# team-charls/charls

Measured on AMD Instinct MI355X. Metric: MPixels/s encode+decode, 4096x4096 8-bit gray, bit-exact vs CharLS, higher is better.
Workload: dtype u8

## Files before the change

charls_amd/batch.py:

```python
from __future__ import annotations

import ctypes as C
from dataclasses import dataclass

import numpy as np

from . import capi


class CodecParams(C.Structure):
    _fields_ = [("frame_info", capi.FrameInfo), ("near_lossless", C.c_int32), ("interleave_mode", C.c_int32),
                ("color_transformation", C.c_int32), ("preset_coding_parameters", capi.PcParameters),
                ("encoding_options", C.c_uint32), ("restart_interval", C.c_uint32)]


class DeviceShard(C.Structure):
    _fields_ = [("device", C.c_int32), ("frame_count", C.c_uint32), ("d_frames", C.c_void_p), ("d_streams", C.c_void_p),
                ("hip_stream", C.c_void_p)]


class Gather(C.Structure):
    _fields_ = [("root_shard", C.c_uint32), ("d_gathered", C.c_void_p), ("capacity_bytes", C.c_size_t),
                ("offsets", C.POINTER(C.c_uint64)), ("total_bytes", C.POINTER(C.c_uint64)), ("transport", C.c_int32)]


TRANSPORT_AUTO, TRANSPORT_RCCL, TRANSPORT_PEER_COPIES = 0, 1, 2


def _bind(lib):
    l = lib.lib
    if getattr(l, "_batch_bound", False):
        return l
    l.charls_amd_encode_batch_device.argtypes = [C.POINTER(CodecParams), C.c_uint32, C.c_void_p, C.c_size_t, C.c_uint32,
                                                 C.c_void_p, C.c_size_t, C.POINTER(C.c_uint64), C.POINTER(C.c_int32),
                                                 C.c_void_p]
    l.charls_amd_encode_batch_device.restype = C.c_int32
    l.charls_amd_decode_batch_device.argtypes = [C.c_uint32, C.c_void_p, C.c_size_t, C.POINTER(C.c_uint64), C.c_void_p,
                                                 C.c_size_t, C.c_uint32, C.POINTER(CodecParams), C.POINTER(C.c_int32),
                                                 C.c_void_p]
    l.charls_amd_decode_batch_device.restype = C.c_int32
    l.charls_amd_last_timings.argtypes = [C.POINTER(C.c_double), C.c_int32]
    l.charls_amd_last_timings.restype = C.c_int32
    l.charls_amd_set_encode_engine.argtypes = [C.c_int32]
    l.charls_amd_set_encode_engine.restype = C.c_int32
    l.charls_amd_set_workspace_limit.argtypes = [C.c_uint64]
    l.charls_amd_set_workspace_limit.restype = C.c_int32
    l.charls_amd_release_work_areas.argtypes = []
    l.charls_amd_release_work_areas.restype = C.c_int32
    l.charls_amd_work_area_bytes.argtypes = []
    l.charls_amd_work_area_bytes.restype = C.c_uint64
    l.charls_amd_encode_batch_devices.argtypes = [C.POINTER(CodecParams), C.c_uint32, C.POINTER(DeviceShard), C.c_size_t,
                                                  C.c_uint32, C.c_size_t, C.POINTER(C.c_uint64), C.POINTER(C.c_int32),
                                                  C.POINTER(Gather)]
    l.charls_amd_encode_batch_devices.restype = C.c_int32
    l.charls_amd_decode_batch_devices.argtypes = [C.c_uint32, C.POINTER(DeviceShard), C.c_size_t, C.POINTER(C.c_uint64),
                                                  C.c_size_t, C.c_uint32, C.POINTER(CodecParams), C.POINTER(C.c_int32)]
    l.charls_amd_decode_batch_devices.restype = C.c_int32
    u64p, i32p, u32p = C.POINTER(C.c_uint64), C.POINTER(C.c_int32), C.POINTER(C.c_uint32)
    l.charls_amd_index_size_bound.argtypes = [C.POINTER(CodecParams), C.c_uint32, C.POINTER(C.c_size_t)]
    l.charls_amd_index_size_bound.restype = C.c_int32
    l.charls_amd_decode_batch_device_and_index.argtypes = [C.c_uint32, C.c_void_p, C.c_size_t, u64p, C.c_void_p, C.c_size_t, C.c_uint32,
                                                           C.c_uint32, C.c_void_p, C.c_size_t, u64p, C.POINTER(CodecParams), i32p,
                                                           C.c_void_p]
    l.charls_amd_decode_batch_device_and_index.restype = C.c_int32
    l.charls_amd_decode_batch_device_indexed.argtypes = [C.c_uint32, C.c_void_p, C.c_size_t, u64p, C.c_void_p, C.c_size_t, u64p,
                                                         C.c_void_p, C.c_size_t, C.c_uint32, C.POINTER(CodecParams), i32p, C.c_void_p]
    l.charls_amd_decode_batch_device_indexed.restype = C.c_int32
    l.charls_amd_decode_rows_batch_device.argtypes = [C.c_uint32, C.c_void_p, C.c_size_t, u64p, C.c_void_p, C.c_size_t, u64p, u32p, u32p,
                                                      C.c_void_p, C.c_size_t, C.c_uint32, i32p, C.c_void_p]
    l.charls_amd_decode_rows_batch_device.restype = C.c_int32
    l.charls_amd_index_counters.argtypes = [u64p, C.c_int32]
    l.charls_amd_index_counters.restype = C.c_int32
    l._batch_bound = True
    return l


def estimated_destination_size(width, height, bits, components) -> int:
    raw = width * height * components * ((bits + 7) // 8)
    return raw + raw // 16 + 1024 + 34


@dataclass
class EncodedBatch:
    streams: "torch.Tensor"
    sizes: np.ndarray
    errcs: np.ndarray
    gpu_ms: tuple


def last_timings(lib=None):
    l = _bind(lib or capi.load_product())
    buf = (C.c_double * 8)()
    n = l.charls_amd_last_timings(buf, 8)
    return tuple(buf[i] for i in range(n))


def encode_batch(frames, *, bits_per_sample=8, component_count=1, interleave_mode=0, near_lossless=0,
                 color_transformation=0, preset=(0, 0, 0, 0, 0), encoding_options=0, restart_interval=0, streams=None,
                 lib=None) -> EncodedBatch:
    import torch
    lib = lib or capi.load_product()
    l = _bind(lib)
    assert frames.is_cuda and frames.is_contiguous()
    count = frames.shape[0]
    if component_count == 1 or interleave_mode == 0:
        height, width = frames.shape[-2], frames.shape[-1]
    else:
        height, width = frames.shape[1], frames.shape[2]
    frame_pitch = frames[0].numel() * frames.element_size()
    if streams is None:
        pitch = (estimated_destination_size(width, height, bits_per_sample, component_count) + 255) & ~255
        streams = torch.empty((count, pitch), dtype=torch.uint8, device=frames.device)
    assert streams.is_contiguous() and streams.shape[0] == count
    p = CodecParams(capi.FrameInfo(width, height, bits_per_sample, component_count), near_lossless, interleave_mode,
                    color_transformation, capi.PcParameters(*preset), encoding_options, restart_interval)
    sizes = np.zeros(count, dtype=np.uint64)
    errcs = np.zeros(count, dtype=np.int32)
    stream = torch.cuda.current_stream(frames.device).cuda_stream
    rc = l.charls_amd_encode_batch_device(C.byref(p), count, frames.data_ptr(), frame_pitch, 0, streams.data_ptr(),
                                          streams.shape[1], sizes.ctypes.data_as(C.POINTER(C.c_uint64)),
                                          errcs.ctypes.data_as(C.POINTER(C.c_int32)), C.c_void_p(stream))
    if rc != 0:
        raise capi.JpegLSError(rc, "charls_amd_encode_batch_device")
    return EncodedBatch(streams, sizes, errcs, last_timings(lib))


def decode_batch(streams, sizes, out, *, lib=None):
    import torch
    lib = lib or capi.load_product()
    l = _bind(lib)
    assert streams.is_cuda and streams.is_contiguous() and out.is_cuda and out.is_contiguous()
    count = streams.shape[0]
    sizes = np.ascontiguousarray(sizes, dtype=np.uint64)
    errcs = np.zeros(count, dtype=np.int32)
    p = CodecParams()
    frame_pitch = out[0].numel() * out.element_size()
    stream = torch.cuda.current_stream(streams.device).cuda_stream
    rc = l.charls_amd_decode_batch_device(count, streams.data_ptr(), streams.shape[1],
                                          sizes.ctypes.data_as(C.POINTER(C.c_uint64)), out.data_ptr(), frame_pitch, 0,
                                          C.byref(p), errcs.ctypes.data_as(C.POINTER(C.c_int32)), C.c_void_p(stream))
    if rc != 0:
        raise capi.JpegLSError(rc, "charls_amd_decode_batch_device")
    return p, errcs, last_timings(lib)



def index_size_bound(width, height, bits_per_sample=8, component_count=1, interleave_mode=0, near_lossless=0,
# ... 237 lines not shown
```

charls_amd/csrc/device/knobs.h:

```cpp
#pragma once
#include <atomic>
#include <climits>
#include <cstdlib>
#include <cstring>
#include <mutex>

namespace jls::knobs {

enum Knob : int
{
    kDecodeGroup = 0,
    kExactDecoder,
    kSequentialIntervals,
    kBlockStuffing,
    kSpecStuffing,
    kJobEvents,
    kWarmEvents,
    kRunJobEvents,
    kRunWarmEvents,
    kRareWarmEvents,
    kTileSamples,
    kPixelMode,
    kSpecChunk,
    kSpecWarm,
    kBatchRounds,
    kCoalesce,
    kCoalesceWaitUs,
    kDecodeWavesPerCu,
    kDecodeWorkgroupWaves,
    kTrace,
    kIdleReleaseMs,
    kNearDecodePixels,
    kCount
};

constexpr long long kUnset = LLONG_MIN;

inline const char* name_of(int k)
{
    static const char* const names[kCount] = {"DECODE_GROUP", "EXACT_DECODER", "SEQUENTIAL_INTERVALS", "BLOCK_STUFFING", "SPEC_STUFFING",
                                              "JOB_EVENTS", "WARM_EVENTS", "RUN_JOB_EVENTS", "RUN_WARM_EVENTS", "RARE_WARM_EVENTS",
                                              "TILE_SAMPLES", "PIXEL_MODE", "SPEC_CHUNK", "SPEC_WARM", "BATCH_ROUNDS", "COALESCE",
                                              "COALESCE_WAIT_US", "DECODE_WAVES_PER_CU", "DECODE_WORKGROUP_WAVES", "TRACE", "IDLE_RELEASE_MS", "NEAR_DECODE_PIXELS"};
    return k >= 0 && k < kCount ? names[k] : nullptr;
}

struct Table
{
    std::atomic<long long> value[kCount];
};

inline long long from_environment(int k)
{
    char name[64] = "CHARLS_AMD_";
    std::strncat(name, name_of(k), sizeof name - std::strlen(name) - 1);
    const char* env = std::getenv(name);
    if (env == nullptr)
        return kUnset;
    return *env == '\0' ? 1 : std::atoll(env);
}

inline Table& table()
{
    static Table* t = [] {
        auto* fresh = new Table;
        for (int k = 0; k < kCount; ++k)
#ifdef JLS_KNOBS_LIVE_ENV
            fresh->value[k].store(kUnset, std::memory_order_relaxed);
#else
            fresh->value[k].store(from_environment(k), std::memory_order_relaxed);
#endif
        return fresh;
    }();
    return *t;
}

inline long long get(Knob k)
{
    const long long v = table().value[k].load(std::memory_order_relaxed);
#ifdef JLS_KNOBS_LIVE_ENV
    if (v == kUnset)
        return from_environment(k);
#endif
    return v;
}

inline bool is_set(Knob k)
{
    return get(k) != kUnset;
}

inline long long get_or(Knob k, long long otherwise)
{
    const long long v = get(k);
    return v == kUnset ? otherwise : v;
}
// ... 18 lines not shown
```

charls_amd/csrc/device/runtime.h:

```cpp
#pragma once
#include <hip/hip_runtime_api.h>

#include <cstddef>
#include <cstdint>

#include "../host/common.h"
#include "scan_types.h"

namespace jls::dev {

charls_jpegls_errc device_status() noexcept;
void require_device();

inline void hip_check(hipError_t e)
{
    if (e != hipSuccess)
        raise(e == hipErrorOutOfMemory ? CHARLS_JPEGLS_ERRC_NOT_ENOUGH_MEMORY : CHARLS_AMD_ERRC_DEVICE_FAILURE);
}

class DeviceBuffer
{
public:
    DeviceBuffer() = default;
    DeviceBuffer(const DeviceBuffer&) = delete;
// ... 85 lines not shown
void launch_find_scan_end(const uint8_t* slots, const MarkerSearch* searches, unsigned long long* found, uint32_t count, hipStream_t stream);
void launch_place_plane_scans(uint8_t* slots, uint64_t slot_pitch, const uint8_t* headers, uint32_t header_size, uint32_t rounds,
                              const uint8_t* private_streams, uint64_t capacity, const ScanResult* results, FrameCursorPod* cursors,
                              uint32_t* redo, uint32_t frames, hipStream_t stream);
void launch_place_epilogue(uint8_t* slots, uint64_t slot_pitch, FrameCursorPod* cursors, bool even_size, uint64_t* sizes,
                           uint32_t* errcs, uint32_t frames, hipStream_t stream);

void set_workspace_limit(uint64_t bytes) noexcept;
uint64_t workspace_limit() noexcept;
void release_shared_work_areas() noexcept;
size_t shared_work_area_bytes() noexcept;
DeviceBuffer& plane_arena();
constexpr int kSeekArenas = 6;
DeviceBuffer& seek_arena(int which);
void* try_ensure(DeviceBuffer& buffer, size_t bytes) noexcept;
void release_work_areas() noexcept;
size_t work_area_bytes() noexcept;
size_t thread_work_area_bytes() noexcept;
void release_thread_work_areas() noexcept;
size_t work_area_budget() noexcept;
uint64_t pipeline_fallback_scans() noexcept;
uint64_t exact_retry_scans() noexcept;

inline size_t with_headroom(size_t bytes) noexcept
{
    size_t v = size_t{64} << 10;
    while (v < bytes)
        v <<= 1;
    return v;
}
size_t shared_areas_keep_bytes() noexcept;

class SharedAreasScope
{
public:
    SharedAreasScope();
    ~SharedAreasScope();
    SharedAreasScope(const SharedAreasScope&) = delete;
    SharedAreasScope& operator=(const SharedAreasScope&) = delete;
    size_t bytes() const noexcept;
    void release() noexcept;

private:
    int device_{0};
};

struct Timings
{
    double values[8];
    int32_t count;
};
Timings& last_timings() noexcept;

constexpr int tile_counter_count = 6;
void speculation_counters(uint64_t out[tile_counter_count]) noexcept;

}
```

charls_amd/csrc/device/runtime.hip:

```cpp
#include <hip/hip_runtime.h>

#include <atomic>
#include <cstdlib>
#include <cstring>
#include <mutex>
#include <vector>

#include "knobs.h"
#include "runtime.h"
#include "scan_serial.hip"
#include "container_kernels.hip"
#include "scan_wave_decode.hip"
#include "pipeline_common.hip"
#include "block_stuffing.hip"
#include "speculative_stuffing.hip"
#include "tile_pipeline.hip"
#include "scan_fast_decode.hip"
#include "scan_group_decode.hip"
#include "group_launch.h"
#include "restart_intervals.hip"
#include "seek_decode.h"

namespace jls::dev {

namespace {
std::once_flag g_once;
charls_jpegls_errc g_status = CHARLS_AMD_ERRC_DEVICE_UNAVAILABLE;
std::atomic<int32_t> g_engine{0};
std::atomic<uint64_t> g_workspace_limit{0};

void probe() noexcept
{
    int count = 0;
    if (hipGetDeviceCount(&count) != hipSuccess || count <= 0)
    {
        (void)hipGetLastError();
        return;
    }
    int device = 0;
    if (hipGetDevice(&device) != hipSuccess)
        return;
    hipDeviceProp_t prop;
    if (hipGetDeviceProperties(&prop, device) != hipSuccess)
        return;
    if (std::strncmp(prop.gcnArchName, "gfx950", 6) != 0 && std::getenv("CHARLS_AMD_ALLOW_ANY_ARCH") == nullptr)
        return;
    g_status = CHARLS_JPEGLS_ERRC_SUCCESS;
}
}

charls_jpegls_errc device_status() noexcept
{
    std::call_once(g_once, probe);
    return g_status;
}

void require_device()
{
    if (device_status() != CHARLS_JPEGLS_ERRC_SUCCESS)
        raise(CHARLS_AMD_ERRC_DEVICE_UNAVAILABLE);
}
// ... 374 lines not shown
        retry_descs[slot] = descs[i];
    }
}

__global__ void scatter_retries(const ScanResult* __restrict__ retry_results, const uint32_t* __restrict__ retry_index,
                                uint32_t retries, ScanResult* __restrict__ results)
{
    const uint32_t s = blockIdx.x * blockDim.x + threadIdx.x;
    if (s < retries)
        results[retry_index[s]] = retry_results[s];
}

template <typename S>
void launch_wave_decode(int nc, const ScanDesc* d_descs, ScanResult* d_results, uint32_t count, size_t lds,
                        hipStream_t stream)
{
    switch (nc)
    {
    case 1:
        hipLaunchKernelGGL((decode_scans_wave<S, 1>), dim3(count), dim3(64), lds, stream, d_descs, d_results);
        break;
    case 2:
        hipLaunchKernelGGL((decode_scans_wave<S, 2>), dim3(count), dim3(64), lds, stream, d_descs, d_results);
        break;
    case 3:
        hipLaunchKernelGGL((decode_scans_wave<S, 3>), dim3(count), dim3(64), lds, stream, d_descs, d_results);
        break;
    default:
        hipLaunchKernelGGL((decode_scans_wave<S, 4>), dim3(count), dim3(64), lds, stream, d_descs, d_results);
        break;
    }
}
}

bool seek_decode_eligible(const ScanDesc& d) noexcept
{
    return d.restart_interval == 0 && wave_decode_eligible(d);
}

uint64_t decode_launch_key(const ScanDesc& d) noexcept
{
    const uint64_t base = (static_cast<uint64_t>(d.width) << 16) | (static_cast<uint64_t>(d.components & 0xFF) << 8) |
                          (static_cast<uint64_t>(d.interleave_mode & 3) << 4) | (d.near_lossless != 0 ? 8u : 0u) |
                          (fast_decode_eligible(d) || pixel_group_lanes(d, 1) != 0 ? 4u : 0u) |
                          (d.bits_per_sample > 8 ? 2u : 0u) | (wave_decode_eligible(d) ? 1u : 0u);
    if (!interval_decode_candidate(d))
        return base;
    return (uint64_t{1} << 63) | (static_cast<uint64_t>(d.restart_interval) << 47) | (static_cast<uint64_t>(d.height) << 31) |
           (static_cast<uint64_t>(d.width & 0xFFFF) << 15) | (static_cast<uint64_t>(d.components & 7) << 12) |
           (static_cast<uint64_t>(d.interleave_mode & 3) << 10) | (base & 15u);
}

namespace {
constexpr int kMaxPipelineLanes = 2;
struct PipelineLanes
{
    hipStream_t streams[kMaxPipelineLanes]{};
    bool created = false;
    int device = -1;
    ~PipelineLanes() { destroy(); }
    void destroy() noexcept
    {
        if (!created)
            return;
        int current = 0;
        const bool switched = hipGetDevice(&current) == hipSuccess && current != device && hipSetDevice(device) == hipSuccess;
        for (hipStream_t s : streams)
            (void)hipStreamDestroy(s);
        if (switched)
            (void)hipSetDevice(current);
        created = false;
    }
    void ensure()
    {
        int current = 0;
        hip_check(hipGetDevice(&current));
        if (created && current == device)
            return;
        destroy();
        for (hipStream_t& s : streams)
            hip_check(hipStreamCreateWithFlags(&s, hipStreamNonBlocking));
        created = true;
        device = current;
    }
};

constexpr int kIntervalArenas = 8;
struct WorkAreas
{
    DeviceBuffer pipeline, plane, interval[kIntervalArenas], seek[kSeekArenas];
    PipelineLanes lanes;
    size_t bytes() const noexcept
    {
        size_t total = pipeline.capacity() + plane.capacity();
        for (const DeviceBuffer& b : interval)
            total += b.capacity();
        for (const DeviceBuffer& b : seek)
            total += b.capacity();
        return total;
    }
    void release() noexcept
    {
        pipeline.release();
        plane.release();
        for (DeviceBuffer& b : interval)
            b.release();
        for (DeviceBuffer& b : seek)
// ... 391 lines not shown
            o = align_up(o + n, 256);
            return at;
        };
        off_keyinv = take(samples * 2);
        off_seg = take(static_cast<size_t>(tiles + 1) * pipe::kChains * 4);
        off_total = take(pipe::kChains * 4);
        off_base = take(pipe::kChains * 4);
        off_jobfirst = take((pipe::kChains + 1) * 4);
        off_planpart = take(static_cast<size_t>(tile::kPlanGroups) * pipe::kChains * 4);
        const uint32_t run_slots = d.bits_per_sample > 8 ? 1u : 2u;
        const size_t slot_bytes = d.bits_per_sample > 8 ? 4 : 2;
        const size_t slots = static_cast<size_t>(tile::slots_capacity(samples, run_slots, lines)) + tile::kSlack;
        off_rec = take(slots * slot_bytes);
        off_code = take(slots * slot_bytes);
        off_jobs = take(max_jobs * sizeof(tile::JobState));
        off_runjobs = take(max_run_jobs * sizeof(tile::RunJob));
        off_bbase = take(static_cast<size_t>(tiles) * 16);
        off_raw = take(raw_bytes);
        off_bits = take(16);
        off_status = take(8);
        off_stuff = take(std::max(block_stuffing_enabled() ? (raw_bytes / pipe::kStuffChunk + 1) * pipe::kStuffWords * 4 : 0,
                                  spec_stuffing_enabled() ? pipe::stuff_spec_table_words(raw_bytes, pipe::stuff_spec_geometry().chunk_bytes) * 4 : 0));
        bytes = o;
    }
};

void ensure_tile_attributes()
{
    static std::mutex guard;
    static uint64_t done[4] = {0, 0, 0, 0};
    int device = 0;
    hip_check(hipGetDevice(&device));
    std::lock_guard<std::mutex> lock(guard);
    if (device >= 0 && device < 256 && (done[device >> 6] >> (device & 63) & 1u) != 0)
        return;
    const int lds = 160 * 1024;
    auto set = [&](const void* kernel) { hip_check(hipFuncSetAttribute(kernel, hipFuncAttributeMaxDynamicSharedMemorySize, lds)); };
    set(reinterpret_cast<const void*>(tile::analyze_tiles<uint8_t, 0>));
    set(reinterpret_cast<const void*>(tile::analyze_tiles<uint16_t, 0>));
    set(reinterpret_cast<const void*>(tile::pack_tiles<uint8_t>));
    set(reinterpret_cast<const void*>(tile::pack_tiles<uint16_t>));
    set(reinterpret_cast<const void*>(tile::sort_tiles<uint8_t, 0>));
    set(reinterpret_cast<const void*>(tile::sort_tiles<uint16_t, 0>));
    set(reinterpret_cast<const void*>(tile::analyze_pixel_tiles<uint8_t>));
    set(reinterpret_cast<const void*>(tile::analyze_pixel_tiles<uint16_t>));
    set(reinterpret_cast<const void*>(tile::sort_pixel_tiles<uint8_t>));
    set(reinterpret_cast<const void*>(tile::sort_pixel_tiles<uint16_t>));
    if (device >= 0 && device < 256)
        done[device >> 6] |= uint64_t{1} << (device & 63);
}

constexpr size_t kCounterBytes = 256;

template <typename S>
void run_tile_pipeline(const ScanDesc& proto, ScanDesc* d_descs, ScanResult* d_results, uint32_t count, hipStream_t stream)
{
    const size_t budget = t_shared_areas != nullptr ? std::min(arena_budget(pipeline_arena().capacity()), shared_areas_keep_bytes())
                                                    : arena_budget(pipeline_arena().capacity());
    TileLayout lay(proto, proto.stream_capacity, count);
    size_t per_scan = lay.bytes + 2 * (sizeof(tile::Work) + sizeof(pipe::Work));
    uint32_t resident = static_cast<uint32_t>(std::max<size_t>(1, std::min<size_t>(count, budget / per_scan)));
    if (resident < count)
    {
        lay = TileLayout(proto, proto.stream_capacity, resident);
        per_scan = lay.bytes + 2 * (sizeof(tile::Work) + sizeof(pipe::Work));
        resident = static_cast<uint32_t>(std::max<size_t>(1, std::min<size_t>(count, budget / per_scan)));
    }
    uint8_t* arena = nullptr;
    const bool over_limit = g_workspace_limit.load() != 0 && budget < per_scan;
    for (; !over_limit;)
    {
        uint32_t room = resident;
        if (t_shared_areas != nullptr)
        {
            room = 1;
            while (room < resident)
                room *= 2;
            room = static_cast<uint32_t>(std::max<size_t>(resident, std::min<size_t>(room, budget / per_scan)));
        }
        arena = static_cast<uint8_t*>(try_ensure(pipeline_arena(), per_scan * room + kCounterBytes));
        if (arena != nullptr || resident == 1)
            break;
        resident = (resident + 1) / 2;
    }
    if (arena == nullptr)
    {
        note_pipeline_fallback(count);
        launch_encode_serial(d_descs, d_results, count, stream);
        last_timings().count = 2;
        return;
    }
    const uint32_t passes = (count + resident - 1) / resident;
    const uint32_t per_pass = (count + passes - 1) / passes;
    auto* d_counters = reinterpret_cast<uint32_t*>(arena + per_scan * resident);
    hip_check(hipMemsetAsync(d_counters, 0, kCounterBytes, stream));
    std::vector<std::vector<tile::Work>> works(passes);
    std::vector<std::vector<pipe::Work>> stuff_works(passes);
    std::vector<StageTimer> timers;
    timers.reserve(passes);
    const bool overlap_stuffing = passes > 1;
    hipStream_t stuff_stream = stream;
    EventList packed, stuffed;
    pipeline_lanes().ensure();
    if (overlap_stuffing)
    {
        stuff_stream = pipeline_lanes().streams[0];
        packed.grow(passes);
        stuffed.grow(passes);
    }
    hipStream_t runs_stream = pipeline_lanes().streams[1];
    EventList sorted(passes), runs_coded(passes);
    ensure_tile_attributes();

    for (uint32_t pass = 0; pass < passes; ++pass)
    {
        const uint32_t first = pass * per_pass;
        const uint32_t n = std::min(per_pass, count - first);
        hipStream_t s = stream;
        const size_t copy = pass & 1u;
        uint8_t* tables = arena + lay.bytes * per_pass;
        auto* d_works = reinterpret_cast<tile::Work*>(tables) + copy * per_pass;
        auto* d_stuff = reinterpret_cast<pipe::Work*>(tables + 2 * sizeof(tile::Work) * per_pass) + copy * per_pass;
        works[pass].resize(n);
        stuff_works[pass].resize(n);
        for (uint32_t i = 0; i < n; ++i)
        {
            uint8_t* base = arena + lay.bytes * i;
            tile::Work& w = works[pass][i];
            w.keyinv = reinterpret_cast<uint16_t*>(base + lay.off_keyinv);
            w.seg = reinterpret_cast<uint32_t*>(base + lay.off_seg);
            w.plan_part = reinterpret_cast<uint32_t*>(base + lay.off_planpart);
            w.chain_total = reinterpret_cast<uint32_t*>(base + lay.off_total);
            w.chain_base = reinterpret_cast<uint32_t*>(base + lay.off_base);
            w.job_first = reinterpret_cast<uint32_t*>(base + lay.off_jobfirst);
            w.rec = reinterpret_cast<uint32_t*>(base + lay.off_rec);
            w.code = reinterpret_cast<uint32_t*>(base + lay.off_code);
            w.jobs = reinterpret_cast<tile::JobState*>(base + lay.off_jobs);
            w.run_jobs = reinterpret_cast<tile::RunJob*>(base + lay.off_runjobs);
            w.run_job_events = lay.run_job_events;
            w.run_warm_events = lay.run_warm_events;
            w.rare_warm_events = lay.rare_warm_events;
            w.blockbase = reinterpret_cast<uint64_t*>(base + lay.off_bbase);
            w.tile_tail = reinterpret_cast<uint64_t*>(base + lay.off_bbase) + lay.tiles;
            w.raw = reinterpret_cast<uint32_t*>(base + lay.off_raw);
            w.raw_words = lay.raw_bytes / 4;
            w.total_bits = reinterpret_cast<uint64_t*>(base + lay.off_bits) + copy;
            w.status = reinterpret_cast<uint32_t*>(base + lay.off_status) + copy;
            w.counters = d_counters;
            w.lines_per_tile = lay.lines_per_tile;
            w.tiles = lay.tiles;
            w.job_events = lay.job_events;
            w.warm_events = lay.warm_events;
            w.segs_per_line = lay.plan.segs_per_line;
            w.seg_pixels = lay.plan.seg_pixels;
            w.tile_capacity = lay.plan.tile_capacity;
            w.run_slots = tile::run_slots_of<S>();
            pipe::Work& sw = stuff_works[pass][i];
            std::memset(&sw, 0, sizeof sw);
            sw.raw = w.raw;
            sw.raw_words = w.raw_words;
            sw.total_bits = w.total_bits;
            sw.status = w.status;
            sw.stuff_tables = reinterpret_cast<uint32_t*>(base + lay.off_stuff);
        }
        hip_check(hipMemcpyAsync(d_works, works[pass].data(), sizeof(tile::Work) * n, hipMemcpyHostToDevice, s));
        hip_check(hipMemcpyAsync(d_stuff, stuff_works[pass].data(), sizeof(pipe::Work) * n, hipMemcpyHostToDevice, s));

        const ScanDesc* descs = d_descs + first;
        const uint32_t tiles_grid = 8 * ((lay.tiles + 7) / 8);
        const tile::TilePlan& plan = lay.plan;
        const bool pixel_mode = plan.mode == 2;
        const size_t lds_a = pixel_mode ? tile::analyze_pixel_lds_bytes(plan.lines_per_tile, plan.step, plan.max_pixels, plan.nc, sizeof(S), plan.tile_capacity)
                                        : tile::analyze_lds_bytes(proto.width, lay.lines_per_tile, sizeof(S), proto.interleave_mode);
        const size_t lds_b = pixel_mode ? tile::sort_pixel_lds_bytes(plan.lines_per_tile, plan.step, plan.max_pixels, plan.nc, sizeof(S), plan.tile_capacity)
                                        : tile::sort_lds_bytes(proto.width, lay.lines_per_tile, sizeof(S), proto.interleave_mode);
        timers.emplace_back(s);
        StageTimer& t = timers.back();
        t.mark();
        if (pixel_mode)
            hipLaunchKernelGGL((tile::analyze_pixel_tiles<S>), dim3(tiles_grid, n), dim3(tile::kThreads), lds_a, s, descs, d_works);
        else
            hipLaunchKernelGGL((tile::analyze_tiles<S, 0>), dim3(tiles_grid, n), dim3(tile::kThreads), lds_a, s, descs, d_works);
        t.mark();
        hipLaunchKernelGGL(tile::sum_chains, dim3(tile::kPlanGroups, n), dim3(tile::kPlanThreads), 0, s, descs, d_works);
        hipLaunchKernelGGL(tile::plan_chains, dim3(n), dim3(tile::kPlanThreads), 0, s, descs, d_works);
        hipLaunchKernelGGL(tile::apply_chains, dim3(tile::kPlanGroups, n), dim3(tile::kPlanThreads), 0, s, descs, d_works);
        if (pixel_mode)
            hipLaunchKernelGGL((tile::sort_pixel_tiles<S>), dim3(tiles_grid, n), dim3(tile::kThreads), lds_b, s, descs, d_works);
        else
            hipLaunchKernelGGL((tile::sort_tiles<S, 0>), dim3(tiles_grid, n), dim3(tile::kThreads), lds_b, s, descs, d_works);
        t.mark();
        hip_check(hipEventRecord(sorted[pass], s));
        hip_check(hipStreamWaitEvent(runs_stream, sorted[pass], 0));
        {
            const uint32_t run_jobs = static_cast<uint32_t>(lay.max_run_jobs);
            const dim3 lanes((static_cast<uint64_t>(run_jobs) * n + 63) / 64);
            const dim3 count_grid(std::min<uint32_t>(run_jobs, std::max<uint32_t>(32, 4096 / n)), n);
            if (pixel_mode)
                hipLaunchKernelGGL((tile::count_runs<S, 1>), count_grid, dim3(64), 0, runs_stream, d_works, plan.nc);
            else
                hipLaunchKernelGGL((tile::count_runs<S, 0>), count_grid, dim3(64), 0, runs_stream, d_works, 1u);
            hipLaunchKernelGGL(tile::scan_runs, dim3(n), dim3(64), 0, runs_stream, d_works);
            if (proto.interleave_mode != 2)
            {
                if (pixel_mode)
                    hipLaunchKernelGGL((tile::compact_rare_runs<S, 1>), count_grid, dim3(64), 0, runs_stream, d_works);
                else
                    hipLaunchKernelGGL((tile::compact_rare_runs<S, 0>), count_grid, dim3(64), 0, runs_stream, d_works);
            }
            const uint32_t rare_blocks = proto.interleave_mode != 2 ? n : 0u;
#define JLS_RUN_CHAIN(ILV, FMT)                                                                                          \
    do                                                                                                                   \
    {                                                                                                                    \
        hipLaunchKernelGGL((tile::warm_run_jobs<S, ILV, FMT>), dim3(rare_blocks + lanes.x), dim3(64), 0, runs_stream, descs, d_works, n, rare_blocks); \
        hipLaunchKernelGGL((tile::walk_run_jobs<S, ILV, FMT>), lanes, dim3(64), 0, runs_stream, descs, d_works, n);      \
        hipLaunchKernelGGL((tile::settle_runs<S, ILV, FMT>), dim3(n), dim3(64), 0, runs_stream, descs, d_works, n);  \
    } while (0)
            if (!pixel_mode)
                JLS_RUN_CHAIN(0, 0);
            else if (proto.interleave_mode == 2)
                JLS_RUN_CHAIN(2, 1);
            else if (proto.interleave_mode == 1)
                JLS_RUN_CHAIN(1, 1);
            else
                JLS_RUN_CHAIN(0, 1);
#undef JLS_RUN_CHAIN
        }
        hip_check(hipEventRecord(runs_coded[pass], runs_stream));
        hipLaunchKernelGGL((tile::walk_jobs<S>), dim3(static_cast<uint32_t>((lay.max_jobs + 63) / 64), n), dim3(64), 0, s, descs, d_works);
        hipLaunchKernelGGL((tile::settle_chains<S>), dim3(pipe::kChains, n), dim3(64), 0, s, descs, d_works, n);
        hip_check(hipStreamWaitEvent(s, runs_coded[pass], 0));
        t.mark();
        if (overlap_stuffing && pass > 0)
            hip_check(hipStreamWaitEvent(s, stuffed[pass - 1], 0));
        hipLaunchKernelGGL(tile::clear_pack_state, dim3(1, n), dim3(256), 0, s, d_works,
                           static_cast<uint32_t>(static_cast<size_t>(lay.tiles) * 16));
        hipLaunchKernelGGL((tile::pack_tiles<S>), dim3(lay.tiles, n), dim3(tile::pack_threads_for(lay.plan.tile_capacity)), tile::pack_lds_bytes(lay.plan.tile_capacity, proto.bits_per_sample), s,
                           descs, d_works);
        t.mark();
        if (overlap_stuffing)
        {
            hip_check(hipEventRecord(packed[pass], s));
            hip_check(hipStreamWaitEvent(stuff_stream, packed[pass], 0));
        }
        t.mark_on(stuff_stream);
        if (block_stuffing_enabled() && n <= kBlockStuffingScans)
        {
            const uint32_t chunk_waves = static_cast<uint32_t>((lay.raw_bytes / pipe::kStuffChunk + 1 + 63) / 64);
            const uint32_t survey_blocks = pipe::stuff_survey_blocks(lay.raw_bytes);
            hipLaunchKernelGGL(pipe::stuff_survey, dim3(survey_blocks, n), dim3(64), 0, stuff_stream, d_stuff);
            hipLaunchKernelGGL(pipe::stuff_resolve, dim3(n), dim3(pipe::kStuffResolveThreads), 0, stuff_stream, d_stuff);
            hipLaunchKernelGGL(pipe::stuff_emit, dim3(chunk_waves, n), dim3(64), 0, stuff_stream, descs, d_stuff, d_results + first);
        }
        else if (spec_stuffing_enabled() && (pass + 1 == passes || lay.raw_bytes >= kSpecStuffingAlwaysBytes))
        {
            const pipe::SpecGeometry spec = pipe::stuff_spec_geometry();
            const uint32_t waves = static_cast<uint32_t>(lay.raw_bytes / spec.chunk_bytes + 1);
            hipLaunchKernelGGL(pipe::stuff_spec_survey, dim3(waves, n), dim3(64), 0, stuff_stream, d_stuff, spec.chunk_bytes, spec.warm_bytes);
            hipLaunchKernelGGL(pipe::stuff_spec_resolve, dim3(n), dim3(64), 0, stuff_stream, d_stuff, spec.chunk_bytes);
            hipLaunchKernelGGL(pipe::stuff_spec_emit, dim3(waves, n), dim3(64), 0, stuff_stream, descs, d_stuff, d_results + first, spec.chunk_bytes);
        }
        else
            hipLaunchKernelGGL(pipe::stuff_scan, dim3(n), dim3(64), 0, stuff_stream, descs, d_stuff, d_results + first);
        t.mark_on(stuff_stream);
        if (overlap_stuffing)
            hip_check(hipEventRecord(stuffed[pass], stuff_stream));
        hip_check(hipGetLastError());
    }
    if (overlap_stuffing)
        hip_check(hipStreamWaitEvent(stream, stuffed[passes - 1], 0));
    static_assert(tile::kCounters == tile_counter_count, "runtime.h: tile_counter_count");
    uint32_t counters[tile::kCounters] = {};
    hip_check(hipMemcpyAsync(counters, d_counters, sizeof counters, hipMemcpyDeviceToHost, stream));
    hip_check(hipStreamSynchronize(stream));
    for (uint32_t i = 0; i < tile::kCounters; ++i)
        g_speculation[i].fetch_add(counters[i]);
#ifdef JLS_PHASE_CLOCKS
    {
        unsigned long long all[(kCounterBytes - 32) / 8] = {};
        hip_check(hipMemcpy(all, reinterpret_cast<const uint8_t*>(d_counters) + 32, sizeof all, hipMemcpyDeviceToHost));
        std::fprintf(stderr, "phase_clocks");
        for (unsigned long long v : all)
            std::fprintf(stderr, " %llu", v);
        std::fprintf(stderr, "\n");
    }
#endif
    Timings& tm = last_timings();
    double stage_ms[5] = {0, 0, 0, 0, 0};
    for (StageTimer& t : timers)
    {
        for (int i = 0; i < 4; ++i)
            stage_ms[i] += t.between(i, i + 1);
        stage_ms[4] += t.between(5, 6);
    }
    for (int i = 0; i < 5; ++i)
        tm.values[2 + i] = stage_ms[i];
    tm.count = 7;
}

}

bool pipeline_eligible(const ScanDesc& d) noexcept
{
    if (encode_engine() == EncodeEngine::serial)
        return false;
    if (d.near_lossless != 0)
        return false;
    const bool planar = d.interleave_mode == 0 && d.components == 1 && d.color_transformation == 0;
    const bool interleaved = d.interleave_mode != 0 && d.components >= 2 && d.components <= 4 &&
                             (d.color_transformation == 0 || d.components == 3);
    if (!planar && !interleaved)
        return false;
    const uint64_t samples = static_cast<uint64_t>(d.width) * d.height * static_cast<uint64_t>(d.components);
    if (samples >= (uint64_t{1} << 31))
        return false;
    if (d.reset == 0 && samples >= (uint64_t{1} << 23))
        return false;
    if (d.bits_per_sample > 8 && ((reinterpret_cast<uintptr_t>(d.pixels) | d.pixel_stride) & 1u) != 0)
        return false;
    return true;
}

namespace {
void launch_encode_intervals(const ScanDesc& proto, ScanDesc* d_descs, ScanResult* d_results, uint32_t count,
                             hipStream_t stream)
{
    const uint32_t lines = proto.restart_interval;
    const uint32_t intervals = (proto.height + lines - 1) / lines;
    ScanDesc sub_proto = proto;
    sub_proto.height = lines;
    sub_proto.restart_interval = 0;
    const size_t worst = worst_case_scan_bytes(proto.width, lines, proto.interleave_mode == 0 ? 1 : proto.components,
                                               proto.bits_per_sample);
    const bool needs_scratch = !pipeline_eligible(sub_proto);
    const size_t scratch_samples = needs_scratch ? line_scratch_samples(proto.width, proto.interleave_mode, proto.components) : 0;
    const size_t first_capacity = std::min(worst, align_up(2 * (static_cast<size_t>(proto.stream_capacity) / intervals) + 4096, 256));
    constexpr size_t kBufferBudget = size_t{8} << 30;
    for (uint32_t first = 0; first < count;)
    {
        size_t capacity = first_capacity;
        uint32_t group = 0;
        for (int attempt = 0; attempt < 2; ++attempt)
        {
            group = static_cast<uint32_t>(std::max<size_t>(1, std::min<size_t>(count - first, kBufferBudget / (capacity * intervals))));
            const size_t subs_n = static_cast<size_t>(group) * intervals;
            auto* d_subs = static_cast<ScanDesc*>(interval_arena(2).ensure(sizeof(ScanDesc) * subs_n));
            auto* d_sub_results = static_cast<ScanResult*>(interval_arena(3).ensure(sizeof(ScanResult) * subs_n));
            auto* d_offsets = static_cast<uint64_t*>(interval_arena(0).ensure(sizeof(uint64_t) * subs_n));
            auto* d_scratch = needs_scratch
                                  ? static_cast<uint16_t*>(interval_arena(5).ensure(sizeof(uint16_t) * scratch_samples * subs_n))
                                  : nullptr;
            auto* d_buffers = static_cast<uint8_t*>(interval_arena(4).ensure(capacity * subs_n));
// ... 270 lines not shown
```

charls_amd/csrc/host/misc_api.cpp:

```cpp
#include <string>
#include <system_error>

#include "../device/knobs.h"
#include "../device/runtime.h"
#include "common.h"
#include "scan_engine.h"

using namespace jls;

namespace {

const char* message_of(int32_t e) noexcept
{
    switch (e)
    {
    case 0: return "Success";
    case 1: return "Not enough memory (host or GPU) to complete the operation";
    case 2: return "A callback function returned a non-zero value";
    case 3: return "The destination buffer is too small to hold all the output";
    case 4: return "The source buffer ends before the JPEG-LS stream is complete";
    case 5: return "The entropy-coded data is not valid JPEG-LS data";
    case 6: return "The stream uses a JPEG encoding other than JPEG-LS";
    case 7: return "The stream uses a parameter value this implementation does not support";
    case 8: return "The colour transformation of the stream is not supported";
// ... 127 lines not shown

charls_jpegls_errc charls_amd_set_workspace_limit(uint64_t bytes)
{
    dev::set_workspace_limit(bytes);
    return CHARLS_JPEGLS_ERRC_SUCCESS;
}

charls_jpegls_errc charls_amd_release_work_areas(void)
{
    dev::release_work_areas();
    release_idle_engine_resources();
    return CHARLS_JPEGLS_ERRC_SUCCESS;
}

uint64_t charls_amd_work_area_bytes(void)
{
    return dev::work_area_bytes();
}

int32_t charls_amd_speculation_counters(uint64_t* out, int32_t capacity)
{
    uint64_t v[dev::tile_counter_count];
    dev::speculation_counters(v);
    int32_t n = 0;
    for (; out != nullptr && n < capacity && n < dev::tile_counter_count; ++n)
        out[n] = v[n];
    return n;
}

int32_t charls_amd_engine_counters(uint64_t* out, int32_t capacity)
{
    uint64_t stats[5], v[10];
    coalescer_stats(stats);
    for (int i = 0; i < 4; ++i)
        v[i] = stats[i];
    v[4] = dev::pipeline_fallback_scans();
    v[5] = stats[4];
    v[6] = idle_engine_resource_bytes();
    v[7] = dev::deferred_free_bytes();
    v[8] = idle_releases();
    v[9] = dev::exact_retry_scans();
    int32_t n = 0;
    for (; out != nullptr && n < capacity && n < 10; ++n)
        out[n] = v[n];
    return n;
}

charls_jpegls_errc charls_amd_debug_set_knob(const char* name, int64_t value)
{
    return knobs::set(name, value == INT64_MIN ? knobs::kUnset : static_cast<long long>(value)) ? CHARLS_JPEGLS_ERRC_SUCCESS
                                                                                                 : CHARLS_JPEGLS_ERRC_INVALID_ARGUMENT;
}

int32_t charls_amd_last_timings(double* out, int32_t capacity)
{
    const dev::Timings& t = dev::last_timings();
    const int32_t n = t.count < capacity ? t.count : capacity;
    for (int32_t i = 0; i < n; ++i)
        out[i] = t.values[i];
    return n;
}

}
```

include/charls_amd.h:

```cpp
#ifndef CHARLS_AMD_H
#define CHARLS_AMD_H

#include <stddef.h>
#include <stdint.h>

#ifdef __cplusplus
extern "C" {
#endif

#if defined(__GNUC__)
#define CHARLS_AMD_API __attribute__((visibility("default")))
#else
#define CHARLS_AMD_API
#endif

typedef int32_t charls_jpegls_errc;
enum
{
    CHARLS_JPEGLS_ERRC_SUCCESS = 0,
    CHARLS_JPEGLS_ERRC_NOT_ENOUGH_MEMORY = 1,
    CHARLS_JPEGLS_ERRC_CALLBACK_FAILED = 2,
    CHARLS_JPEGLS_ERRC_DESTINATION_TOO_SMALL = 3,
    CHARLS_JPEGLS_ERRC_NEED_MORE_DATA = 4,
    CHARLS_JPEGLS_ERRC_INVALID_DATA = 5,
// ... 304 lines not shown
CHARLS_AMD_API void charls_amd_devices_destroy(charls_amd_devices* context);
CHARLS_AMD_API charls_jpegls_errc charls_amd_devices_encode_batch(charls_amd_devices* context, const charls_amd_codec_params* params,
                                                                  uint32_t shard_count, const charls_amd_device_shard* shards,
                                                                  size_t frame_pitch_bytes, uint32_t stride,
                                                                  size_t stream_pitch_bytes, uint64_t* sizes,
                                                                  charls_jpegls_errc* errcs, const charls_amd_gather* gather);
CHARLS_AMD_API charls_jpegls_errc charls_amd_devices_decode_batch(charls_amd_devices* context, uint32_t shard_count,
                                                                  const charls_amd_device_shard* shards, size_t stream_pitch_bytes,
                                                                  const uint64_t* sizes, size_t frame_pitch_bytes, uint32_t stride,
                                                                  charls_amd_codec_params* params_out, charls_jpegls_errc* errcs);
CHARLS_AMD_API uint64_t charls_amd_devices_work_area_bytes(charls_amd_devices* context);
CHARLS_AMD_API charls_jpegls_errc charls_amd_devices_release_work_areas(charls_amd_devices* context);

CHARLS_AMD_API charls_jpegls_errc charls_amd_jpegls_encoder_set_restart_interval(charls_jpegls_encoder* encoder,
                                                                                 uint32_t lines);

CHARLS_AMD_API charls_jpegls_errc charls_amd_jpegls_decoder_get_index_size(const charls_jpegls_decoder* decoder,
                                                                           uint32_t lines_per_seek_point, size_t* bytes);
CHARLS_AMD_API charls_jpegls_errc charls_amd_jpegls_decoder_decode_to_buffer_and_index(
    charls_jpegls_decoder* decoder, void* destination_buffer, size_t destination_size_bytes, uint32_t stride,
    uint32_t lines_per_seek_point, void* index, size_t index_capacity, size_t* index_bytes);
CHARLS_AMD_API charls_jpegls_errc charls_amd_jpegls_decoder_set_index(charls_jpegls_decoder* decoder, const void* index,
                                                                      size_t index_size_bytes);
CHARLS_AMD_API charls_jpegls_errc charls_amd_jpegls_decoder_decode_rows(charls_jpegls_decoder* decoder, uint32_t first_row,
                                                                        uint32_t row_count, void* destination_buffer,
                                                                        size_t destination_size_bytes, uint32_t stride);
CHARLS_AMD_API int32_t charls_amd_index_counters(uint64_t* out, int32_t capacity);

CHARLS_AMD_API charls_jpegls_errc charls_amd_index_size_bound(const charls_amd_codec_params* params,
                                                              uint32_t lines_per_seek_point, size_t* bytes);
CHARLS_AMD_API charls_jpegls_errc charls_amd_decode_batch_device_and_index(
    uint32_t frame_count, const void* d_streams, size_t stream_pitch_bytes, const uint64_t* sizes, void* d_frames,
    size_t frame_pitch_bytes, uint32_t stride, uint32_t lines_per_seek_point, void* indexes, size_t index_pitch_bytes,
    uint64_t* index_sizes, charls_amd_codec_params* params_out, charls_jpegls_errc* errcs, void* hip_stream);
CHARLS_AMD_API charls_jpegls_errc charls_amd_decode_batch_device_indexed(
    uint32_t frame_count, const void* d_streams, size_t stream_pitch_bytes, const uint64_t* sizes, const void* indexes,
    size_t index_pitch_bytes, const uint64_t* index_sizes, void* d_frames, size_t frame_pitch_bytes, uint32_t stride,
    charls_amd_codec_params* params_out, charls_jpegls_errc* errcs, void* hip_stream);
CHARLS_AMD_API charls_jpegls_errc charls_amd_decode_rows_batch_device(
    uint32_t frame_count, const void* d_streams, size_t stream_pitch_bytes, const uint64_t* sizes, const void* indexes,
    size_t index_pitch_bytes, const uint64_t* index_sizes, const uint32_t* first_rows, const uint32_t* row_counts,
    void* d_bands, size_t band_pitch_bytes, uint32_t stride, charls_jpegls_errc* errcs, void* hip_stream);

CHARLS_AMD_API charls_jpegls_errc charls_amd_set_encode_engine(int32_t engine);

CHARLS_AMD_API charls_jpegls_errc charls_amd_set_workspace_limit(uint64_t bytes);
CHARLS_AMD_API charls_jpegls_errc charls_amd_release_work_areas(void);
CHARLS_AMD_API uint64_t charls_amd_work_area_bytes(void);

CHARLS_AMD_API int32_t charls_amd_engine_counters(uint64_t* out, int32_t capacity);

CHARLS_AMD_API charls_jpegls_errc charls_amd_debug_set_knob(const char* name, int64_t value);

CHARLS_AMD_API int32_t charls_amd_last_timings(double* out, int32_t capacity);

CHARLS_AMD_API int32_t charls_amd_speculation_counters(uint64_t* out, int32_t capacity);

CHARLS_AMD_API charls_jpegls_errc charls_amd_device_status(void);

#ifdef __cplusplus
}
#endif
#endif
```

Before: 16310.

## Add optional two-lane encode pipeline schedule with staggered pass start

```diff
diff --git a/charls_amd/batch.py b/charls_amd/batch.py
--- a/charls_amd/batch.py
+++ b/charls_amd/batch.py
@@ -71,6 +71,8 @@
     l.charls_amd_decode_rows_batch_device.restype = C.c_int32
     l.charls_amd_index_counters.argtypes = [u64p, C.c_int32]
     l.charls_amd_index_counters.restype = C.c_int32
+    l.charls_amd_debug_last_encode_plan.argtypes = [u32p]
+    l.charls_amd_debug_last_encode_plan.restype = None
     l._batch_bound = True
     return l
 
@@ -93,6 +95,13 @@
     buf = (C.c_double * 8)()
     n = l.charls_amd_last_timings(buf, 8)
     return tuple(buf[i] for i in range(n))
+
+
+def last_encode_plan(lib=None) -> dict:
+    l = _bind(lib or capi.load_product())
+    buf = (C.c_uint32 * 4)()
+    l.charls_amd_debug_last_encode_plan(buf)
+    return {"passes": buf[0], "lanes": buf[1], "scans_per_pass": buf[2], "streams": buf[3]}
 
 
 def encode_batch(frames, *, bits_per_sample=8, component_count=1, interleave_mode=0, near_lossless=0,
diff --git a/charls_amd/csrc/device/encode_schedule.h b/charls_amd/csrc/device/encode_schedule.h
--- /dev/null
+++ b/charls_amd/csrc/device/encode_schedule.h
@@ -0,0 +1,57 @@
+#pragma once
+#include <cstdint>
+#include <vector>
+
+namespace jls::schedule {
+
+constexpr int32_t kNone = -1;
+
+struct Pass
+{
+    uint32_t first, n;
+    uint32_t lane;
+    uint32_t slot_first, slots;
+    uint32_t copy;
+    int32_t after_packed;
+    int32_t after_stuffed;
+    int32_t after_stagger;
+};
+
+struct Plan
+{
+    uint32_t lanes = 1, per_pass = 0;
+    std::vector<Pass> passes;
+};
+
+inline Plan plan_passes(uint32_t count, uint32_t resident, uint32_t lanes)
+{
+    Plan plan;
+    if (count == 0)
+        return plan;
+    if (resident == 0)
+        resident = 1;
+    plan.lanes = lanes == 2 && count >= 2 && resident >= 2 ? 2u : 1u;
+    const uint32_t room = plan.lanes == 2 ? resident / 2 : resident;
+    uint32_t passes = (count + room - 1) / room;
+    if (passes < plan.lanes)
+        passes = plan.lanes;
+    plan.per_pass = (count + passes - 1) / passes;
+    for (uint32_t k = 0, first = 0; first < count; ++k, first += plan.per_pass)
+    {
+        Pass p{};
+        p.first = first;
+        p.n = count - first < plan.per_pass ? count - first : plan.per_pass;
+        p.lane = k % plan.lanes;
+        p.slot_first = p.lane * room;
+        p.slots = plan.per_pass;
+        p.copy = (k / plan.lanes) & 1u;
+        const int32_t before = static_cast<int32_t>(k) - static_cast<int32_t>(plan.lanes);
+        p.after_packed = before >= 0 ? before : kNone;
+        p.after_stuffed = before >= 0 ? before : kNone;
+        p.after_stagger = plan.lanes == 2 && k == 1 ? 0 : kNone;
+        plan.passes.push_back(p);
+    }
+    return plan;
+}
+
+}
diff --git a/charls_amd/csrc/device/knobs.h b/charls_amd/csrc/device/knobs.h
--- a/charls_amd/csrc/device/knobs.h
+++ b/charls_amd/csrc/device/knobs.h
@@ -31,6 +31,8 @@
     kTrace,
     kIdleReleaseMs,
     kNearDecodePixels,
+    kEncodeLanes,
+    kEncodeStagger,
     kCount
 };
 
@@ -41,7 +43,8 @@
     static const char* const names[kCount] = {"DECODE_GROUP", "EXACT_DECODER", "SEQUENTIAL_INTERVALS", "BLOCK_STUFFING", "SPEC_STUFFING",
                                               "JOB_EVENTS", "WARM_EVENTS", "RUN_JOB_EVENTS", "RUN_WARM_EVENTS", "RARE_WARM_EVENTS",
                                               "TILE_SAMPLES", "PIXEL_MODE", "SPEC_CHUNK", "SPEC_WARM", "BATCH_ROUNDS", "COALESCE",
-                                              "COALESCE_WAIT_US", "DECODE_WAVES_PER_CU", "DECODE_WORKGROUP_WAVES", "TRACE", "IDLE_RELEASE_MS", "NEAR_DECODE_PIXELS"};
+                                              "COALESCE_WAIT_US", "DECODE_WAVES_PER_CU", "DECODE_WORKGROUP_WAVES", "TRACE", "IDLE_RELEASE_MS", "NEAR_DECODE_PIXELS",
+                                              "ENCODE_LANES", "ENCODE_STAGGER"};
     return k >= 0 && k < kCount ? names[k] : nullptr;
 }
 
diff --git a/charls_amd/csrc/device/runtime.h b/charls_amd/csrc/device/runtime.h
--- a/charls_amd/csrc/device/runtime.h
+++ b/charls_amd/csrc/device/runtime.h
@@ -161,6 +161,8 @@
 };
 Timings& last_timings() noexcept;
 
+void last_encode_plan(uint32_t out[4]) noexcept;
+
 constexpr int tile_counter_count = 6;
 void speculation_counters(uint64_t out[tile_counter_count]) noexcept;
 
diff --git a/charls_amd/csrc/device/runtime.hip b/charls_amd/csrc/device/runtime.hip
--- a/charls_amd/csrc/device/runtime.hip
+++ b/charls_amd/csrc/device/runtime.hip
@@ -7,6 +7,7 @@
 #include <vector>
 
 #include "knobs.h"
+#include "encode_schedule.h"
 #include "runtime.h"
 #include "scan_serial.hip"
 #include "container_kernels.hip"
@@ -487,7 +488,7 @@
 }
 
 namespace {
-constexpr int kMaxPipelineLanes = 2;
+constexpr int kMaxPipelineLanes = 3;
 struct PipelineLanes
 {
     hipStream_t streams[kMaxPipelineLanes]{};
@@ -985,6 +986,12 @@
 
 constexpr size_t kCounterBytes = 256;
 
+uint32_t* last_plan_note() noexcept
+{
+    static thread_local uint32_t note[4] = {0, 0, 0, 0};
+    return note;
+}
+
 template <typename S>
 void run_tile_pipeline(const ScanDesc& proto, ScanDesc* d_descs, ScanResult* d_results, uint32_t count, hipStream_t stream)
 {
@@ -999,6 +1006,9 @@
         per_scan = lay.bytes + 2 * (sizeof(tile::Work) + sizeof(pipe::Work));
         resident = static_cast<uint32_t>(std::max<size_t>(1, std::min<size_t>(count, budget / per_scan)));
     }
+    const size_t works_bytes = align_up(sizeof(tile::Work) * count, 256);
+    const size_t tables_bytes = works_bytes + align_up(sizeof(pipe::Work) * count, 256);
+    auto tables_room = [&](uint32_t scans) { return (per_scan - lay.bytes) * scans; };
     uint8_t* arena = nullptr;
     const bool over_limit = g_workspace_limit.load() != 0 && budget < per_scan;
     for (; !over_limit;)
@@ -1011,7 +1021,8 @@
                 room *= 2;
             room = static_cast<uint32_t>(std::max<size_t>(resident, std::min<size_t>(room, budget / per_scan)));
         }
-        arena = static_cast<uint8_t*>(try_ensure(pipeline_arena(), per_scan * room + kCounterBytes));
+        arena = static_cast<uint8_t*>(try_ensure(pipeline_arena(), per_scan * room + kCounterBytes +
+                                                                       (tables_bytes > tables_room(resident) ? tables_bytes : 0)));
         if (arena != nullptr || resident == 1)
             break;
         resident = (resident + 1) / 2;
@@ -1021,45 +1032,24 @@
         note_pipeline_fallback(count);
         launch_encode_serial(d_descs, d_results, count, stream);
         last_timings().count = 2;
-        return;
-    }
-    const uint32_t passes = (count + resident - 1) / resident;
-    const uint32_t per_pass = (count + passes - 1) / passes;
+        std::memset(last_plan_note(), 0, 4 * sizeof(uint32_t));
+        return;
+    }
+    const bool two_lanes = t_shared_areas == nullptr && knobs::get_or(knobs::kEncodeLanes, 1) == 2;
+    const schedule::Plan plan_of_call = schedule::plan_passes(count, resident, two_lanes ? 2u : 1u);
+    const uint32_t passes = static_cast<uint32_t>(plan_of_call.passes.size());
+    const uint32_t per_pass = plan_of_call.per_pass;
     auto* d_counters = reinterpret_cast<uint32_t*>(arena + per_scan * resident);
     hip_check(hipMemsetAsync(d_counters, 0, kCounterBytes, stream));
-    std::vector<std::vector<tile::Work>> works(passes);
-    std::vector<std::vector<pipe::Work>> stuff_works(passes);
-    std::vector<StageTimer> timers;
-    timers.reserve(passes);
-    const bool overlap_stuffing = passes > 1;
-    hipStream_t stuff_stream = stream;
-    EventList packed, stuffed;
-    pipeline_lanes().ensure();
-    if (overlap_stuffing)
-    {
-        stuff_stream = pipeline_lanes().streams[0];
-        packed.grow(passes);
-        stuffed.grow(passes);
-    }
-    hipStream_t runs_stream = pipeline_lanes().streams[1];
-    EventList sorted(passes), runs_coded(passes);
-    ensure_tile_attributes();
-
-    for (uint32_t pass = 0; pass < passes; ++pass)
-    {
-        const uint32_t first = pass * per_pass;
-        const uint32_t n = std::min(per_pass, count - first);
-        hipStream_t s = stream;
-        const size_t copy = pass & 1u;
-        uint8_t* tables = arena + lay.bytes * per_pass;
-        auto* d_works = reinterpret_cast<tile::Work*>(tables) + copy * per_pass;
-        auto* d_stuff = reinterpret_cast<pipe::Work*>(tables + 2 * sizeof(tile::Work) * per_pass) + copy * per_pass;
-        works[pass].resize(n);
-        stuff_works[pass].resize(n);
-        for (uint32_t i = 0; i < n; ++i)
-        {
-            uint8_t* base = arena + lay.bytes * i;
-            tile::Work& w = works[pass][i];
+    uint8_t* d_tables = tables_bytes > tables_room(resident) ? arena + per_scan * resident + kCounterBytes : arena + lay.bytes * resident;
+    std::vector<uint8_t> host_tables(tables_bytes);
+    auto* works = reinterpret_cast<tile::Work*>(host_tables.data());
+    auto* stuff_works = reinterpret_cast<pipe::Work*>(host_tables.data() + works_bytes);
+    for (const schedule::Pass& p : plan_of_call.passes)
+        for (uint32_t i = 0; i < p.n; ++i)
+        {
+            uint8_t* base = arena + lay.bytes * (p.slot_first + i);
+            tile::Work w{};
             w.keyinv = reinterpret_cast<uint16_t*>(base + lay.off_keyinv);
             w.seg = reinterpret_cast<uint32_t*>(base + lay.off_seg);
             w.plan_part = reinterpret_cast<uint32_t*>(base + lay.off_planpart);
@@ -1077,8 +1067,8 @@
             w.tile_tail = reinterpret_cast<uint64_t*>(base + lay.off_bbase) + lay.tiles;
             w.raw = reinterpret_cast<uint32_t*>(base + lay.off_raw);
             w.raw_words = lay.raw_bytes / 4;
-            w.total_bits = reinterpret_cast<uint64_t*>(base + lay.off_bits) + copy;
-            w.status = reinterpret_cast<uint32_t*>(base + lay.off_status) + copy;
+            w.total_bits = reinterpret_cast<uint64_t*>(base + lay.off_bits) + p.copy;
+            w.status = reinterpret_cast<uint32_t*>(base + lay.off_status) + p.copy;
             w.counters = d_counters;
             w.lines_per_tile = lay.lines_per_tile;
             w.tiles = lay.tiles;
@@ -1088,16 +1078,59 @@
             w.seg_pixels = lay.plan.seg_pixels;
             w.tile_capacity = lay.plan.tile_capacity;
             w.run_slots = tile::run_slots_of<S>();
-            pipe::Work& sw = stuff_works[pass][i];
+            pipe::Work sw;
             std::memset(&sw, 0, sizeof sw);
             sw.raw = w.raw;
             sw.raw_words = w.raw_words;
             sw.total_bits = w.total_bits;
             sw.status = w.status;
             sw.stuff_tables = reinterpret_cast<uint32_t*>(base + lay.off_stuff);
-        }
-        hip_check(hipMemcpyAsync(d_works, works[pass].data(), sizeof(tile::Work) * n, hipMemcpyHostToDevice, s));
-        hip_check(hipMemcpyAsync(d_stuff, stuff_works[pass].data(), sizeof(pipe::Work) * n, hipMemcpyHostToDevice, s));
+            std::memcpy(works + p.first + i, &w, sizeof w);
+            std::memcpy(stuff_works + p.first + i, &sw, sizeof sw);
+        }
+    hip_check(hipMemcpyAsync(d_tables, host_tables.data(), tables_bytes, hipMemcpyHostToDevice, stream));
+    std::vector<StageTimer> timers;
+    timers.reserve(passes);
+    const bool overlap_stuffing = passes > 1;
+    hipStream_t stuff_stream = stream;
+    EventList packed, stuffed;
+    pipeline_lanes().ensure();
+    if (overlap_stuffing)
+    {
+        stuff_stream = pipeline_lanes().streams[0];
+        packed.grow(passes);
+        stuffed.grow(passes);
+    }
+    hipStream_t runs_stream = pipeline_lanes().streams[1];
+    EventList sorted(passes), runs_coded(passes);
+    hipStream_t lane_streams[2] = {stream, stream};
+    EventList lane_events(plan_of_call.lanes == 2 ? 2 : 0);
+    if (plan_of_call.lanes == 2)
+    {
+        lane_streams[1] = pipeline_lanes().streams[2];
+        hip_check(hipEventRecord(lane_events[0], stream));
+        hip_check(hipStreamWaitEvent(lane_streams[1], lane_events[0], 0));
+    }
+    const long long stagger_at = knobs::get_or(knobs::kEncodeStagger, 1);
+    {
+        uint32_t* note = last_plan_note();
+        note[0] = passes;
+        note[1] = plan_of_call.lanes;
+        note[2] = per_pass;
+        note[3] = 2u + (overlap_stuffing ? 1u : 0u) + (plan_of_call.lanes == 2 ? 1u : 0u);
+    }
+    ensure_tile_attributes();
+
+    for (uint32_t pass = 0; pass < passes; ++pass)
+    {
+        const schedule::Pass& sp = plan_of_call.passes[pass];
+        const uint32_t first = sp.first;
+        const uint32_t n = sp.n;
+        hipStream_t s = lane_streams[sp.lane];
+        auto* d_works = reinterpret_cast<tile::Work*>(d_tables) + first;
+        auto* d_stuff = reinterpret_cast<pipe::Work*>(d_tables + works_bytes) + first;
+        if (sp.after_stagger != schedule::kNone)
+            hip_check(hipStreamWaitEvent(s, lane_events[1], 0));
 
         const ScanDesc* descs = d_descs + first;
         const uint32_t tiles_grid = 8 * ((lay.tiles + 7) / 8);
@@ -1115,6 +1148,8 @@
         else
             hipLaunchKernelGGL((tile::analyze_tiles<S, 0>), dim3(tiles_grid, n), dim3(tile::kThreads), lds_a, s, descs, d_works);
         t.mark();
+        if (pass == 0 && plan_of_call.lanes == 2 && stagger_at == 0)
+            hip_check(hipEventRecord(lane_events[1], s));
         hipLaunchKernelGGL(tile::sum_chains, dim3(tile::kPlanGroups, n), dim3(tile::kPlanThreads), 0, s, descs, d_works);
         hipLaunchKernelGGL(tile::plan_chains, dim3(n), dim3(tile::kPlanThreads), 0, s, descs, d_works);
         hipLaunchKernelGGL(tile::apply_chains, dim3(tile::kPlanGroups, n), dim3(tile::kPlanThreads), 0, s, descs, d_works);
@@ -1124,6 +1159,8 @@
             hipLaunchKernelGGL((tile::sort_tiles<S, 0>), dim3(tiles_grid, n), dim3(tile::kThreads), lds_b, s, descs, d_works);
         t.mark();
         hip_check(hipEventRecord(sorted[pass], s));
+        if (pass == 0 && plan_of_call.lanes == 2 && stagger_at != 0 && stagger_at != 2)
+            hip_check(hipEventRecord(lane_events[1], s));
         hip_check(hipStreamWaitEvent(runs_stream, sorted[pass], 0));
         {
             const uint32_t run_jobs = static_cast<uint32_t>(lay.max_run_jobs);
@@ -1162,10 +1199,12 @@
         hip_check(hipEventRecord(runs_coded[pass], runs_stream));
         hipLaunchKernelGGL((tile::walk_jobs<S>), dim3(static_cast<uint32_t>((lay.max_jobs + 63) / 64), n), dim3(64), 0, s, descs, d_works);
         hipLaunchKernelGGL((tile::settle_chains<S>), dim3(pipe::kChains, n), dim3(64), 0, s, descs, d_works, n);
+        if (pass == 0 && plan_of_call.lanes == 2 && stagger_at == 2)
+            hip_check(hipEventRecord(lane_events[1], s));
         hip_check(hipStreamWaitEvent(s, runs_coded[pass], 0));
         t.mark();
-        if (overlap_stuffing && pass > 0)
-            hip_check(hipStreamWaitEvent(s, stuffed[pass - 1], 0));
+        if (sp.after_stuffed != schedule::kNone)
+            hip_check(hipStreamWaitEvent(s, stuffed[sp.after_stuffed], 0));
         hipLaunchKernelGGL(tile::clear_pack_state, dim3(1, n), dim3(256), 0, s, d_works,
                            static_cast<uint32_t>(static_cast<size_t>(lay.tiles) * 16));
         hipLaunchKernelGGL((tile::pack_tiles<S>), dim3(lay.tiles, n), dim3(tile::pack_threads_for(lay.plan.tile_capacity)), tile::pack_lds_bytes(lay.plan.tile_capacity, proto.bits_per_sample), s,
@@ -1231,6 +1270,11 @@
     tm.count = 7;
 }
 
+}
+
+void last_encode_plan(uint32_t out[4]) noexcept
+{
+    std::memcpy(out, last_plan_note(), 4 * sizeof(uint32_t));
 }
 
 bool pipeline_eligible(const ScanDesc& d) noexcept
diff --git a/charls_amd/csrc/host/misc_api.cpp b/charls_amd/csrc/host/misc_api.cpp
--- a/charls_amd/csrc/host/misc_api.cpp
+++ b/charls_amd/csrc/host/misc_api.cpp
@@ -203,6 +203,12 @@
                                                                                                  : CHARLS_JPEGLS_ERRC_INVALID_ARGUMENT;
 }
 
+void charls_amd_debug_last_encode_plan(uint32_t out[4])
+{
+    if (out != nullptr)
+        dev::last_encode_plan(out);
+}
+
 int32_t charls_amd_last_timings(double* out, int32_t capacity)
 {
     const dev::Timings& t = dev::last_timings();
diff --git a/include/charls_amd.h b/include/charls_amd.h
--- a/include/charls_amd.h
+++ b/include/charls_amd.h
@@ -380,6 +380,8 @@
 
 CHARLS_AMD_API charls_jpegls_errc charls_amd_debug_set_knob(const char* name, int64_t value);
 
+CHARLS_AMD_API void charls_amd_debug_last_encode_plan(uint32_t out[4]);
+
 CHARLS_AMD_API int32_t charls_amd_last_timings(double* out, int32_t capacity);
 
 CHARLS_AMD_API int32_t charls_amd_speculation_counters(uint64_t* out, int32_t capacity);
```

New measurement: 16300, median of 2. No clear change (-0.0%).
